# GregVS/Racing-SLAM

Measured on AMD Instinct MI355X. Metric: match+triangulate+local-BA passes/sec @ 2k kpts/frame, 20-KF×10k-pt window, higher is better.
Workload: dtype u8 Hamming (match), f64 (DLT SVD, BA), f32 (gates)

## Files before the change

racing-slam_amd/csrc/ba_solve_body.h:

```cpp
#pragma once
#include "ba_common.h"
#include "ba_backsub_body.h"

#define K7_THREADS 512
#ifndef K7_CHAIN_SIMDS
#define K7_CHAIN_SIMDS 1
#endif
#ifndef K7_V2
#define K7_V2 0
#endif
#if K7_CHAIN_SIMDS == 2
#define K7_TPW 9
#define K7_NTW 4
#else
#define K7_TPW 6
#define K7_NTW 6
#endif

typedef __attribute__((ext_vector_type(4))) double d4;

__device__ __forceinline__ double readlane_f64(double v, int lane)
{
    const int lo = __builtin_amdgcn_readlane(__double2loint(v), lane);
    const int hi = __builtin_amdgcn_readlane(__double2hiint(v), lane);
    return __hiloint2double(hi, lo);
}

__device__ __forceinline__ double fast_rcp(double x)
{
    double r = __builtin_amdgcn_rcp(x);
    const double e = fma(-x, r, 1.0);
    return fma(r, e, r);
}


template <bool HANDOFF, bool ROUND = false>
static __device__ __forceinline__ void ba_reduced_solve_lds_body(const BaDims& d, const BaBufs& b, const BaOpt& opt, const int it = 0,
                                                                 const int n_items = 0)
{
    extern __shared__ __attribute__((aligned(16))) double sm[];
    const int n = d.n, tid = threadIdx.x, nt = K7_THREADS;
    const int set = blockIdx.x;
    const int LD = n + 1 + ((n & 1) ? 1 : 0);
    double* A = sm;
    double* lam = A + (size_t)(n + 1) * LD;
    double* xs = lam + n;
    double* Minv = xs + n;
    double* Us = Minv + 6 * n;
    double* gcs = Us + 6 * n;
    double* grs = gcs + n;
    double* Pd = sm + (((size_t)(n + 1) * LD + 17 * (size_t)n + 1) & ~(size_t)1);
    double* Nf = Pd + 8 * 128;
    __shared__ BaState st;
    __shared__ int s_fail;
    __shared__ double red[K7_THREADS / 64];
    __shared__ double red3[K7_THREADS / 64][3];
    BA_STAMP_DECL;
    const int lane = tid & 63;
    const int wave = __builtin_amdgcn_readfirstlane(tid >> 6);
    const int lr = lane & 15, lq = lane >> 4;
    const int NTL = (n + 1 + 15) / 16;
#if K7_CHAIN_SIMDS == 2
    const bool chain = wave < 2;
    const bool idle = wave == 4 || wave == 5;
    const int tw = (wave & 1) + 2 * (wave >> 2);
    const int cw = wave;
#elif K7_V2
    const bool chain = (wave & 3) == 0;
    const bool idle = false;
    const int tw = chain ? 0 : wave - 1 - (wave >> 2);
#else
    const bool chain = (wave & 3) == 0;
    const bool idle = false;
    const int tw = chain ? 0 : wave - 1 - (wave >> 2);
    const int cw = wave >> 2;
#endif
    int tr[K7_TPW], tc[K7_TPW];
    bool tv[K7_TPW];
#pragma unroll
    for (int s = 0; s < K7_TPW; s++) {
        const int t = K7_NTW * s + tw;
        int r = 0;
#pragma unroll
        for (int q = 1; q < 8; q++) r += (t >= q * (q + 1) / 2) ? 1 : 0;
        tr[s] = r;
        tc[s] = t - r * (r + 1) / 2;
        tv[s] = !chain && !idle && r < NTL;
    }

    auto acc_ld = [&](const double* p) -> double { return ROUND ? ba_load_sc1(p) : *p; };
    if (ROUND) {
#if RS_STAMPS
        if (tid == 0 && set == 0) b.dbg[45] = wall_clock64();
#endif
        if (tid == 0) s_fail = 0;
        const BaState s0 = ba_round_state(b, opt, it, &st, set == 0);
        if (s0.done || set >= s0.nact) return;
        __shared__ unsigned s_lost;
        if (tid == 0) {
            const unsigned long long want = (unsigned long long)(unsigned)s0.n_rounds * (unsigned long long)n_items;
            const unsigned long long t0 = wall_clock64();
            unsigned lost = 0;
            while (ba_load_word_sc1(b.dbg + BA_SDONE) < want) {
                if (wall_clock64() - t0 > b.hand_timeout) { lost = 1; break; }
                __builtin_amdgcn_s_sleep(2);
            }
            s_lost = lost;
#if RS_STAMPS
            if (set == 0) b.dbg[44] = wall_clock64();
#endif
        }
        __syncthreads();
        if (s_lost) {
            if (tid == 0) {
                atomicAdd(b.dbg + BA_HAND_ERR, 1ull);
                const unsigned long long w = ((unsigned long long)(unsigned)s0.n_rounds << 2) | 2ull;
                ba_store_word_sc1(b.dbg + BA_HAND_TAKEN + set, w);
            }
            return;
        }
    }
    if (!ROUND && tid == 0) { st = *b.st; s_fail = 0; }
    double pre_cost = 0.0, pre_fail = 0.0, pre_gm = 0.0;
    if (tid < 64) {
        pre_cost = acc_ld(&b.scal[(size_t)tid * BA_SLOT_STRIDE + 0]);
        pre_fail = acc_ld(&b.scal[(size_t)tid * BA_SLOT_STRIDE + 1 + set]);
        for (int r = 0; r < b.gmax_blocks; r++)
            pre_gm = fmax(pre_gm, acc_ld(&b.gmax_all[((size_t)r * BA_NSLOT + tid) * BA_SLOT_STRIDE]));
    }
    const double pre_sc = tid < n ? b.sc[tid] : 1.0;
    double fold[2] = {0.0, 0.0}, keep[2] = {0.0, 0.0};
#pragma unroll
    for (int h = 0; h < 2; h++) {
        const int i = tid + h * nt;
        if (i < 8 * n) {
            const size_t addr = i < n ? (size_t)set * n + i : (size_t)(b.ns - 1) * n + i;
#pragma unroll
            for (int r = 0; r < BA_UREP; r++) fold[h] += acc_ld(&b.rhs[(size_t)r * b.cam_stride + addr]);
            if (i >= n) keep[h] = b.Ukeep[i - n];
        }
    }
    double sv[K7_TPW][4];
#pragma unroll
    for (int s = 0; s < K7_TPW; s++) {
#pragma unroll
        for (int q = 0; q < 4; q++) sv[s][q] = 0.0;
        if (!tv[s]) continue;
        const int kc = min(16 * tc[s] + lr, n - 1);
#pragma unroll
        for (int q = 0; q < 4; q++) {
            const int ic = min(16 * tr[s] + lq + 4 * q, n - 1);
            const double* sp = b.S + ((size_t)set * n + kc) * n + ic;
            double v = acc_ld(sp);
            for (int r = 1; r < b.srep; r++) v += acc_ld(sp + (size_t)r * b.s_rep_stride);
            sv[s][q] = v;
        }
    }
    __syncthreads();
    if (st.done || set >= st.nact) return;
#if RS_STAMPS
    if (HANDOFF && tid == 0 && set == 0) b.dbg[42] = wall_clock64();
#endif
    const unsigned long long epoch = (unsigned long long)(unsigned)st.n_rounds << 2;
    auto publish = [&](int word, unsigned long long code) {
        if (HANDOFF) {
            asm volatile("s_waitcnt vmcnt(0)" ::: "memory");
            __syncthreads();
            if (tid == 0) {
#if RS_STAMPS
                if (set == 0) b.dbg[word == BA_HAND ? 40 : 43] = wall_clock64();
#endif
                ba_store_word_sc1(b.dbg + word + set, epoch | code);
            }
        }
    };
    BA_STAMP(b, 2);
    for (int i = tid; i < BA_NSLOT * BA_SLOT_STRIDE; i += nt) {
        double* z = b.pt_scal + (size_t)set * BA_NSLOT * BA_SLOT_STRIDE + i;
        if (HANDOFF) ba_store_sc1(z, 0.0);
        else *z = 0.0;
    }
    for (int i = tid; i < 2 * 8 * 128; i += nt) Pd[i] = 0.0;
#if K7_V2
    for (int i = tid; i < (n + 1) * LD; i += nt) A[i] = 0.0;
#endif
#pragma unroll
    for (int h = 0; h < 2; h++) {
        const int i = tid + h * nt;
        if (i < 8 * n) {
            const double v = (i < n || st.fresh) ? fold[h] : keep[h];
            if (i >= n && st.fresh && set == 0) b.Ukeep[i - n] = v;
            if (i < n) grs[i] = v;
            else if (i < n + 6 * n) Us[i - n] = v;
            else gcs[i - 7 * n] = v;
        }
    }
    __syncthreads();
    for (int i = tid; i < n; i += nt) grs[i] += gcs[i];
    if (tid < n) {
        const double h = Us[(tid / 6) * 36 + (tid % 6) * 7];
        double sc = pre_sc;
        if (!st.have_scale) {
            sc = opt.jacobi ? 1.0 / (1.0 + sqrt(h)) : 1.0;
            if (set == 0) b.sc[tid] = sc;
        }
        const double s2 = sc * sc;
        lam[tid] = clampd(s2 * h, opt.dmin, opt.dmax) / (ba_set_radius(st, set) * s2);
    }
    BA_STAMP(b, 3);

    const double fail_sum = wave_sum(pre_fail);
    if (st.fresh) {
        const double c = wave_sum(pre_cost);
        const double gslots = wave_max_nonneg(pre_gm);
        double gm = 0.0;
        for (int i = tid; i < n; i += nt) gm = fmax(gm, fabs(gcs[i]));
        gm = wave_max_nonneg(gm);
        if ((tid & 63) == 0) red[tid >> 6] = gm;
        __syncthreads();
        if (tid == 0) {
            st.x_cost = c;
            if (st.iter == 0) st.initial_cost = st.x_cost;
            double g = gslots;
            for (int w = 0; w < nt / 64; w++) g = fmax(g, red[w]);
            if (!isfinite(st.x_cost)) { st.done = 1; st.termination = RS_BA_FAILURE; }
            else if (g <= opt.gtol) { st.done = 1; st.termination = RS_BA_CONVERGENCE_GRADIENT; }
        }
        __syncthreads();
        if (st.done) { if (tid == 0 && set == 0) *b.st = st; publish(BA_HAND_TAKEN, 2ull); return; }
    } else {
        __syncthreads();
    }
    publish(BA_HAND_TAKEN, 0ull);
    if (tid == 0 && fail_sum > 0.0) s_fail = 1;
    BA_STAMP(b, 0);

    const int NB = n / 6;
#if K7_V2
#if K7_V2 == 2
#define K7_RING(J_) ((J_) % 3)
#else
#define K7_RING(J_) 0
#endif
    double* const Dg0 = Pd;
    double* const Pds0 = Pd + 108;
    double* const ddv = Pd + 216;
    volatile int* const dflag = (volatile int*)(Pd + 232);
    volatile int* const cflag = dflag + 2;
    volatile int* const tflag = dflag + 4;
    auto wait_for = [&](volatile int* word, int want) {
        int spins = 0;
        while (*word < want) {
            if (++spins > (1 << 20)) { s_fail = 1; break; }
            __builtin_amdgcn_s_sleep(1);
        }
    };
    if (chain) {
        BA_STAMP(b, 1);
        const int sl = wave >> 2;
        const int i = 64 * sl + lane, ic = min(i, n);
        double Fp[6];
#pragma unroll
        for (int e = 0; e < 6; e++) Fp[e] = 0.0;
#if RS_STAMPS
        const unsigned long long cpre_ = wall_clock64();
#endif
        __syncthreads();
#if RS_STAMPS
        if (tid == 0 && blockIdx.x == 0) b.dbg[22] += wall_clock64() - cpre_;
#endif
#if RS_STAMPS >= 2
        unsigned long long cs_[6] = {0, 0, 0, 0, 0, 0}, ct_ = wall_clock64();
#define K7_CSTAMP(i) do { if (tid == 0 && blockIdx.x == 0) { const unsigned long long t__ = wall_clock64(); cs_[i] += t__ - ct_; ct_ = t__; } } while (0)
#else
#define K7_CSTAMP(i) do { } while (0)
#endif
        for (int J = 0; J < NB; J++) {
            const int c0 = 6 * J, r0 = c0 + 6;
            double* const Dg = Dg0 + 36 * K7_RING(J);
            double* const Pds = Pds0 + 36 * K7_RING(J);
            const double* const Pdp = Pds0 + 36 * K7_RING(J + 2);
            if (64 * sl + 63 < c0 || 64 * sl > n) {
#if K7_V2 == 2
                if (lane == 0) cflag[sl] = NB + 1;
                break;
#else
                __syncthreads();
                continue;
#endif
            }
#if K7_V2 == 2
            {
                const int other = sl ^ 1;
#pragma unroll
                for (int t = 0; t < K7_NTW; t++) wait_for(tflag + t, J);
                const bool other_owns = (c0 >> 6) == other || ((c0 + 5) >> 6) == other;
                wait_for(cflag + other, other_owns ? J : J - 1);
                __builtin_amdgcn_fence(__ATOMIC_ACQUIRE, "wavefront");
            }
#endif
            double x[6];
#pragma unroll
            for (int k = 0; k < 6; k++) x[k] = A[ic * LD + c0 + k];
            if (J > 0) {
                const double2* g2 = reinterpret_cast<const double2*>(Pdp);
#pragma unroll
                for (int e = 0; e < 6; e++) {
                    const double2 g01 = g2[3 * e], g23 = g2[3 * e + 1], g45 = g2[3 * e + 2];
                    x[0] -= Fp[e] * g01.x; x[1] -= Fp[e] * g01.y; x[2] -= Fp[e] * g23.x;
                    x[3] -= Fp[e] * g23.y; x[4] -= Fp[e] * g45.x; x[5] -= Fp[e] * g45.y;
                }
            }
            K7_CSTAMP(0);
            {
                const int a = i - c0;
                const int o_lo = c0 >> 6, o_hi = (c0 + 5) >> 6;
                if (a >= 0 && a < 6) {
#pragma unroll
                    for (int k = 0; k < 6; k++) Dg[a * 6 + k] = x[k];
                }
                if (sl == o_lo || sl == o_hi) {
                    __builtin_amdgcn_fence(__ATOMIC_RELEASE, "wavefront");
                    __builtin_amdgcn_s_waitcnt(0xc07f);
                    if (lane == 0) dflag[sl] = J + 1;
                }
                const int other = sl ^ 1;
                if (other == o_lo || other == o_hi) {
                    while (dflag[other] < J + 1) { }
                }
                __builtin_amdgcn_fence(__ATOMIC_ACQUIRE, "wavefront");
                __builtin_amdgcn_s_waitcnt(0xc07f);
            }
            double Lm[6][6];
#pragma unroll
            for (int a = 0; a < 6; a++)
#pragma unroll
                for (int e = 0; e <= a; e++) Lm[a][e] = Dg[a * 6 + e];
            K7_CSTAMP(1);
            double dinv[6], dpiv[6];
            bool fbad = false;
#pragma unroll
            for (int c = 0; c < 6; c++) {
                const double piv = Lm[c][c];
                if (!(piv > 0.0) || !isfinite(piv)) fbad = true;
                const double rd = fast_rcp(piv);
                dinv[c] = rd;
                dpiv[c] = piv;
                double lc[6];
#pragma unroll
                for (int a = c + 1; a < 6; a++) lc[a] = Lm[a][c] * rd;
#pragma unroll
                for (int a = c + 1; a < 6; a++)
#pragma unroll
                    for (int e = c + 1; e <= a; e++) Lm[a][e] -= lc[a] * Lm[e][c];
#pragma unroll
                for (int a = c + 1; a < 6; a++) Lm[a][c] = lc[a];
            }
            K7_CSTAMP(2);
            double F[6];
            {
                double t[6];
#pragma unroll
                for (int r = 0; r < 6; r++) {
                    double sacc = x[r];
#pragma unroll
                    for (int e = 0; e < r; e++) sacc -= t[e] * Lm[r][e];
                    t[r] = sacc;
                }
#pragma unroll
                for (int r = 0; r < 6; r++) F[r] = t[r] * dinv[r];
            }
            K7_CSTAMP(3);
            if (i >= c0 && i <= n) {
#pragma unroll
                for (int r = 0; r < 6; r++) A[i * LD + c0 + r] = F[r];
            }
            if (J + 1 < NB) {
                const int k0 = i - r0;
                if (k0 >= 0 && k0 < 6) {
#pragma unroll
                    for (int e = 0; e < 6; e++) Pds[e * 6 + k0] = F[e] * dpiv[e];
                }
                if (lane == 0 && sl == (c0 >> 6)) {
#pragma unroll
                    for (int e = 0; e < 6; e++) ddv[(J & 1) * 8 + e] = dpiv[e];
                }
            }
#pragma unroll
            for (int e = 0; e < 6; e++) Fp[e] = F[e];
            if (lane == 0 && fbad) s_fail = 1;
            K7_CSTAMP(4);
#if K7_V2 == 2
            __builtin_amdgcn_fence(__ATOMIC_RELEASE, "wavefront");
            __builtin_amdgcn_s_waitcnt(0xc07f);
            if (lane == 0) cflag[sl] = J + 1;
#else
            __syncthreads();
#endif
            K7_CSTAMP(5);
        }
#if K7_V2 == 2
        if (lane == 0 && cflag[sl] < NB) cflag[sl] = NB + 1;
#endif
#if RS_STAMPS >= 2
        if (tid == 0 && blockIdx.x == 0) { for (int q = 0; q < 6; q++) b.dbg[16 + q] += cs_[q]; }
#endif
#if RS_STAMPS
        if (tid == 0 && blockIdx.x == 0) { const unsigned long long t__ = wall_clock64(); b.dbg[30] += t__ - cpre_; b.dbg[23] = t__; b.dbg[31] += 1ull; }
#endif
    } else {
        d4 acc[K7_TPW];
#pragma unroll
        for (int s = 0; s < K7_TPW; s++) {
            acc[s] = d4{0.0, 0.0, 0.0, 0.0};
            if (!tv[s]) continue;
            const int k = 16 * tc[s] + lr;
            if (tr[s] >= tc[s] + 2 && 16 * tr[s] + 15 < n) {
#pragma unroll
                for (int q = 0; q < 4; q++) acc[s][q] = (k < n) ? sv[s][q] : 0.0;
                continue;
            }
            const int kc = min(k, n - 1), kb = kc / 6;
            const double gv = grs[kc];
#pragma unroll
            for (int q = 0; q < 4; q++) {
                const int i = 16 * tr[s] + lq + 4 * q;
                const int ic = min(i, n - 1);
                const double uv = Us[kb * 36 + (kc - 6 * kb) * 6 + ic % 6];
                double val = sv[s][q] + ((kb == ic / 6) ? uv : 0.0) + ((i == k) ? lam[ic] : 0.0);
                val = (k < n && i < n && k <= i) ? val : ((i == n && k < n) ? gv : 0.0);
                acc[s][q] = val;
            }
        }
        int paddr[K7_TPW];
        unsigned pmask[K7_TPW];
#pragma unroll
        for (int s = 0; s < K7_TPW; s++) {
            const int k = 16 * tc[s] + lr;
            paddr[s] = (16 * tr[s] + lq) * LD + k;
            unsigned m = 0;
#pragma unroll
            for (int q = 0; q < 4; q++) {
                const int i = 16 * tr[s] + lq + 4 * q;
                m |= (i >= k && i <= n) ? (1u << q) : 0u;
            }
            pmask[s] = m;
        }
        const int LD4 = 4 * LD;
#pragma unroll
        for (int s = 0; s < K7_TPW; s++) {
            if (!tv[s] || tc[s] != 0) continue;
            if (lr >= 6) continue;
#pragma unroll
            for (int q = 0; q < 4; q++)
                if (pmask[s] >> q & 1) A[paddr[s] + q * LD4] = acc[s][q];
        }
        int arow[K7_TPW], brow[K7_TPW];
#pragma unroll
        for (int s = 0; s < K7_TPW; s++) { arow[s] = min(16 * tr[s] + lr, n) * LD; brow[s] = min(16 * tc[s] + lr, n) * LD; }
        const int e1 = min(4 + lq, 5);
        const bool pad1 = lq >= 2;
        __syncthreads();
        for (int J = 0; J < NB; J++) {
            const int c0 = 6 * J, r0 = c0 + 6;
            if (J > 0) {
#if K7_V2 == 2
                wait_for(cflag + 0, J);
                wait_for(cflag + 1, J);
                __builtin_amdgcn_fence(__ATOMIC_ACQUIRE, "wavefront");
#endif
                const int cm = c0 - 6;
                const double* dv = ddv + ((J - 1) & 1) * 8;
                const double d0 = dv[lq], d1 = dv[4 + lq];
#pragma unroll
                for (int s = 0; s < K7_TPW; s++) {
                    if (!tv[s] || 16 * tc[s] + 15 < c0) continue;
                    const double a0 = A[arow[s] + cm + lq], a1 = A[arow[s] + cm + e1];
                    const double b0 = A[brow[s] + cm + lq], b1 = A[brow[s] + cm + e1];
                    acc[s] = __builtin_amdgcn_mfma_f64_16x16x4f64(-a0, b0 * d0, acc[s], 0, 0, 0);
                    acc[s] = __builtin_amdgcn_mfma_f64_16x16x4f64(pad1 ? 0.0 : -a1, b1 * d1, acc[s], 0, 0, 0);
                }
            }
            if (J + 1 < NB) {
#pragma unroll
                for (int s = 0; s < K7_TPW; s++) {
                    if (!tv[s] || 16 * tc[s] + 15 < r0 || 16 * tc[s] >= r0 + 6) continue;
                    const int k = 16 * tc[s] + lr;
                    if (k < r0 || k >= r0 + 6) continue;
#pragma unroll
                    for (int q = 0; q < 4; q++)
                        if (pmask[s] >> q & 1) A[paddr[s] + q * LD4] = acc[s][q];
                }
            }
#if K7_V2 == 2
            __builtin_amdgcn_fence(__ATOMIC_RELEASE, "wavefront");
            __builtin_amdgcn_s_waitcnt(0xc07f);
            if (lane == 0) tflag[tw] = J + 1;
#else
            __syncthreads();
#endif
        }
    }
#else
    if (chain) {
        BA_STAMP(b, 1);
        const int crow = cw * 64 + lane;
#if RS_STAMPS
        const unsigned long long cpre_ = wall_clock64();
#endif
        __syncthreads();
#if RS_STAMPS
        if (tid == 0 && blockIdx.x == 0) b.dbg[22] += wall_clock64() - cpre_;
#endif
        for (int J = 0; J < NB; J++) {
            const int c0 = 6 * J, r0 = c0 + 6;
            const int irow = r0 + crow;
            const bool has_row = irow <= n;
            if (wave != 0 && r0 + 64 > n) {
                __syncthreads();
                __syncthreads();
                continue;
            }
            double* row = A + min(irow, n) * LD + c0;
            double L[6][6], rr[6];
#pragma unroll
            for (int a = 0; a < 6; a++)
#pragma unroll
                for (int e = 0; e <= a; e++) L[a][e] = A[(c0 + a) * LD + c0 + e];
#pragma unroll
            for (int e = 0; e < 6; e++) rr[e] = row[e];
            double dinv[6], dpiv[6], F[6];
            bool fbad = false;
#pragma unroll
            for (int c = 0; c < 6; c++) {
                const double piv = L[c][c];
                if (!(piv > 0.0) || !isfinite(piv)) fbad = true;
                const double rd = fast_rcp(piv);
                dinv[c] = rd;
                dpiv[c] = piv;
                double lc[6];
#pragma unroll
                for (int a = c + 1; a < 6; a++) lc[a] = L[a][c] * rd;
#pragma unroll
                for (int a = c + 1; a < 6; a++)
#pragma unroll
                    for (int e = c + 1; e <= a; e++) L[a][e] -= lc[a] * L[e][c];
#pragma unroll
                for (int a = c + 1; a < 6; a++) L[a][c] = lc[a];
            }
            {
                double t[6];
#pragma unroll
                for (int r = 0; r < 6; r++) {
                    double sacc = rr[r];
#pragma unroll
                    for (int e = 0; e < r; e++) sacc -= t[e] * L[r][e];
                    t[r] = sacc;
                }
#pragma unroll
                for (int r = 0; r < 6; r++) F[r] = t[r] * dinv[r];
            }
            if (has_row) {
#pragma unroll
                for (int r = 0; r < 6; r++) {
                    row[r] = F[r];
                    Nf[r * 128 + irow] = -F[r];
                    Pd[r * 128 + irow] = F[r] * dpiv[r];
                }
            }
            __syncthreads();
            if (J + 1 < NB) {
                double* nxt = row + 6;
                double x[6];
#pragma unroll
                for (int k = 0; k < 6; k++) x[k] = nxt[k];
#pragma unroll
                for (int e = 0; e < 6; e++) {
                    const double2* g2 = reinterpret_cast<const double2*>(Pd + e * 128 + r0);
                    const double2 g01 = g2[0], g23 = g2[1], g45 = g2[2];
                    x[0] -= F[e] * g01.x; x[1] -= F[e] * g01.y;
                    x[2] -= F[e] * g23.x; x[3] -= F[e] * g23.y;
                    x[4] -= F[e] * g45.x; x[5] -= F[e] * g45.y;
                }
                if (has_row) {
#pragma unroll
                    for (int k = 0; k < 6; k++) nxt[k] = x[k];
                }
            }
            if (tid == 63) {
#pragma unroll
                for (int a = 1; a < 6; a++)
#pragma unroll
                    for (int e = 0; e < a; e++) Minv[J * 36 + a * 6 + e] = L[a][e];
                if (fbad) s_fail = 1;
            }
            __syncthreads();
        }
#if RS_STAMPS
        if (tid == 0 && blockIdx.x == 0) { const unsigned long long t__ = wall_clock64(); b.dbg[30] += t__ - cpre_; b.dbg[23] = t__; b.dbg[31] += 1ull; }
#endif
    } else {
        d4 acc[K7_TPW];
        double opA[K7_TPW][2], opB[K7_TPW][2];
#pragma unroll
        for (int s = 0; s < K7_TPW; s++) {
            acc[s] = d4{0.0, 0.0, 0.0, 0.0};
            opA[s][0] = opA[s][1] = opB[s][0] = opB[s][1] = 0.0;
            if (!tv[s]) continue;
            const int k = 16 * tc[s] + lr;
            if (tr[s] >= tc[s] + 2 && 16 * tr[s] + 15 < n) {
#pragma unroll
                for (int q = 0; q < 4; q++) acc[s][q] = (k < n) ? sv[s][q] : 0.0;
                continue;
            }
            const int kc = min(k, n - 1), kb = kc / 6;
            const double gv = grs[kc];
#pragma unroll
            for (int q = 0; q < 4; q++) {
                const int i = 16 * tr[s] + lq + 4 * q;
                const int ic = min(i, n - 1);
                const double uv = Us[kb * 36 + (kc - 6 * kb) * 6 + ic % 6];
                double val = sv[s][q] + ((kb == ic / 6) ? uv : 0.0) + ((i == k) ? lam[ic] : 0.0);
                val = (k < n && i < n && k <= i) ? val : ((i == n && k < n) ? gv : 0.0);
                acc[s][q] = val;
            }
        }
#pragma unroll
        for (int s = 0; s < K7_TPW; s++) {
            if (!tv[s] || tc[s] != 0) continue;
            const int k = lr;
            if (k >= 6) continue;
#pragma unroll
            for (int q = 0; q < 4; q++) {
                const int i = 16 * tr[s] + lq + 4 * q;
                if (i >= k && i <= n) A[i * LD + k] = acc[s][q];
            }
        }
        int paddr[K7_TPW];
        unsigned pmask[K7_TPW];
#pragma unroll
        for (int s = 0; s < K7_TPW; s++) {
            const int k = 16 * tc[s] + lr;
            paddr[s] = (16 * tr[s] + lq) * LD + k;
            unsigned m = 0;
#pragma unroll
            for (int q = 0; q < 4; q++) {
                const int i = 16 * tr[s] + lq + 4 * q;
                m |= (i >= k && i <= n) ? (1u << q) : 0u;
            }
            pmask[s] = m;
        }
        const int LD4 = 4 * LD;
        __syncthreads();
        for (int J = 0; J < NB; J++) {
            const int c0 = 6 * J, r0 = c0 + 6;
            if (J > 0) {
#pragma unroll
                for (int s = 1; s < K7_TPW; s += 2) {
                    if (!tv[s] || 16 * tc[s] + 15 < c0) continue;
                    acc[s] = __builtin_amdgcn_mfma_f64_16x16x4f64(opA[s][0], opB[s][0], acc[s], 0, 0, 0);
                    acc[s] = __builtin_amdgcn_mfma_f64_16x16x4f64(opA[s][1], opB[s][1], acc[s], 0, 0, 0);
                }
            }
            if (J + 1 < NB) {
#pragma unroll
                for (int s = 0; s < K7_TPW; s++) {
                    if (!tv[s] || 16 * tc[s] + 15 < r0 || 16 * tc[s] >= r0 + 6) continue;
                    const int k = 16 * tc[s] + lr;
                    if (k < r0 || k >= r0 + 6) continue;
#pragma unroll
                    for (int q = 0; q < 4; q++)
                        if (pmask[s] >> q & 1) A[paddr[s] + q * LD4] = acc[s][q];
                }
            }
            __syncthreads();
            if (J + 1 < NB) {
#pragma unroll
                for (int s = 0; s < K7_TPW; s++) {
                    if (!tv[s] || 16 * tc[s] + 15 < r0) continue;
#pragma unroll
                    for (int kc = 0; kc < 2; kc++) {
                        opA[s][kc] = Nf[(4 * kc + lq) * 128 + 16 * tr[s] + lr];
                        opB[s][kc] = Pd[(4 * kc + lq) * 128 + 16 * tc[s] + lr];
                    }
                }
#pragma unroll
                for (int s = 0; s < K7_TPW; s += 2) {
                    if (!tv[s] || 16 * tc[s] + 15 < r0) continue;
                    acc[s] = __builtin_amdgcn_mfma_f64_16x16x4f64(opA[s][0], opB[s][0], acc[s], 0, 0, 0);
                    acc[s] = __builtin_amdgcn_mfma_f64_16x16x4f64(opA[s][1], opB[s][1], acc[s], 0, 0, 0);
                }
            }
            __syncthreads();
        }
    }
#endif
    __syncthreads();
    if (s_fail) {
        if (tid == 0) {
            if (set == 0) { st.solver_failed = 1; *b.st = st; }
            else b.set_out[set].solver_failed = 1;
        }
        publish(BA_HAND, 1ull);
        return;
    }
    if (wave == 0) {
        const double* yrow = A + (size_t)n * LD;
        double y0 = yrow[min(lane, n)], y1 = yrow[min(64 + lane, n)];
        const int i0 = min(lane, n), i1 = min(64 + lane, n);
#define K7_BS_LOAD(J_, L_, P0_, P1_)                                                                       \
    {                                                                                                      \
        const int jj_ = max((J_), 0), cc_ = 6 * jj_;                                                       \
        _Pragma("unroll") for (int e = 1; e < 6; e++)                                                      \
            _Pragma("unroll") for (int t = 0; t < e; t++) L_[e][t] = K7_V2 ? A[(cc_ + e) * LD + cc_ + t] : Minv[jj_ * 36 + e * 6 + t]; \
        _Pragma("unroll") for (int e = 0; e < 6; e++) P0_[e] = A[(cc_ + e) * LD + i0];                     \
        if (cc_ > 64) { _Pragma("unroll") for (int e = 0; e < 6; e++) P1_[e] = A[(cc_ + e) * LD + i1]; }   \
    }
#define K7_BS_STEP(J_, L_, P0_, P1_)                                                                       \
    {                                                                                                      \
        const int c0_ = 6 * (J_);                                                                          \
        double x[6];                                                                                       \
        _Pragma("unroll") for (int t = 5; t >= 0; t--) {                                                   \
            const int idx = c0_ + t;                                                                       \
            double sacc = readlane_f64(idx >= 64 ? y1 : y0, idx & 63);                                     \
            _Pragma("unroll") for (int e = 5; e > t; e--) sacc -= L_[e][t] * x[e];                         \
            x[t] = sacc;                                                                                   \
        }                                                                                                  \
        _Pragma("unroll") for (int e = 0; e < 6; e++) y0 -= P0_[e] * x[e];                                 \
        if (c0_ > 64) { _Pragma("unroll") for (int e = 0; e < 6; e++) y1 -= P1_[e] * x[e]; }               \
        if (lane == 0) { _Pragma("unroll") for (int t = 0; t < 6; t++) xs[c0_ + t] = x[t]; }               \
    }
        double La[6][6], Pa0[6], Pa1[6], Lb[6][6], Pb0[6], Pb1[6];
        K7_BS_LOAD(NB - 1, La, Pa0, Pa1);
        for (int J = NB - 1; J >= 0; J -= 2) {
            K7_BS_LOAD(J - 1, Lb, Pb0, Pb1);
            K7_BS_STEP(J, La, Pa0, Pa1);
            if (J - 1 >= 0) {
                K7_BS_LOAD(J - 2, La, Pa0, Pa1);
                K7_BS_STEP(J - 1, Lb, Pb0, Pb1);
            }
        }
#undef K7_BS_LOAD
#undef K7_BS_STEP
    }
    __syncthreads();
    BA_STAMP(b, 6);
#if RS_STAMPS
    if (tid == 0 && blockIdx.x == 0) { b.dbg[25] += wall_clock64() - b.dbg[23]; }
#endif
    double* dc_set = b.dc + (size_t)set * BA_DC_STRIDE(n);
    if (HANDOFF) {
        int badi = 0;
        for (int i = tid; i < n; i += nt) {
            const double dlt = -xs[i];
            if (!isfinite(dlt)) badi = 1;
            ba_store_sc1(&dc_set[i], dlt);
        }
        publish(BA_HAND, __syncthreads_or(badi) ? 1ull : 0ull);
    }
    double mcc = 0.0, ssq = 0.0, xsq = 0.0;
    bool bad = false;
    const double* Xc = b.Xc + (size_t)st.cur * d.C * 6;
    const int cand = (st.cur + 1 + set) % (b.ns + 1);
    double* Xn = b.Xc + (size_t)cand * d.C * 6;
    for (int c = tid; c < d.C; c += nt) {
        const int s = b.slot[c];
        bool active = false;
        if (s >= 0)
            for (int k = 0; k < 6; k++) active = active || Us[s * 36 + k * 7] > 0.0;
        for (int k = 0; k < 6; k++) {
            const double x = Xc[6 * c + k];
            if (s >= 0) {
                const double dlt = -xs[6 * s + k];
                if (!isfinite(dlt)) bad = true;
                mcc += 0.5 * (dlt * dlt * lam[6 * s + k] - dlt * gcs[6 * s + k]);
                const double xn = x + dlt;
                if (active) { ssq += (x - xn) * (x - xn); xsq += x * x; }
                Xn[6 * c + k] = xn;
                if (!HANDOFF) dc_set[6 * s + k] = dlt;
            } else {
                Xn[6 * c + k] = x;
            }
        }
        cam_prepare(Xn + 6 * c, b.prep + ((size_t)cand * d.C + c) * BA_PREP);
    }
    mcc = wave_sum(mcc); ssq = wave_sum(ssq); xsq = wave_sum(xsq);
    if (__any(bad) && (tid & 63) == 0) s_fail = 1;
    if ((tid & 63) == 0) { red3[tid >> 6][0] = mcc; red3[tid >> 6][1] = ssq; red3[tid >> 6][2] = xsq; }
    __syncthreads();
    if (tid == 0) {
        double a0 = 0, a1 = 0, a2 = 0;
        for (int w = 0; w < nt / 64; w++) { a0 += red3[w][0]; a1 += red3[w][1]; a2 += red3[w][2]; }
        if (set == 0) {
            st.cam_scal[0] = a0; st.cam_scal[1] = a1; st.cam_scal[2] = a2;
            st.solver_failed = s_fail;
            *b.st = st;
        } else {
            BaSetOut so;
            so.cam_scal[0] = a0; so.cam_scal[1] = a1; so.cam_scal[2] = a2; so.cam_scal[3] = 0.0;
            so.solver_failed = s_fail;
#pragma unroll
            for (int q = 0; q < 7; q++) so.pad[q] = 0;
            b.set_out[set] = so;
        }
    }
    BA_STAMP(b, 7);
    BA_STAMP_FLUSH(b, 0);
}
```

Before: 1998.

## Precompute block-scaled off-diagonal columns in parallel before single-wave back-substitution

```diff
diff --git a/racing-slam_amd/csrc/ba_solve_body.h b/racing-slam_amd/csrc/ba_solve_body.h
--- a/racing-slam_amd/csrc/ba_solve_body.h
+++ b/racing-slam_amd/csrc/ba_solve_body.h
@@ -704,44 +704,78 @@
         publish(BA_HAND, 1ull);
         return;
     }
+    for (int idx = tid; idx < NB * (n + 1); idx += nt) {
+        const int J = idx / (n + 1), c = idx - J * (n + 1), c0 = 6 * J;
+        if (c < c0 + 6) continue;
+        double q[6];
+#pragma unroll
+        for (int a = 0; a < 6; a++) q[a] = A[c * LD + c0 + a];
+#pragma unroll
+        for (int a = 4; a >= 0; a--)
+#pragma unroll
+            for (int e = 5; e > a; e--) q[a] -= (K7_V2 ? A[(c0 + e) * LD + c0 + a] : Minv[J * 36 + e * 6 + a]) * q[e];
+#pragma unroll
+        for (int a = 0; a < 6; a++) A[(c0 + a) * LD + c] = q[a];
+    }
+    __syncthreads();
     if (wave == 0) {
-        const double* yrow = A + (size_t)n * LD;
-        double y0 = yrow[min(lane, n)], y1 = yrow[min(64 + lane, n)];
-        const int i0 = min(lane, n), i1 = min(64 + lane, n);
-#define K7_BS_LOAD(J_, L_, P0_, P1_)                                                                       \
+        const double* q0row = A + (size_t)min(lane, n) * LD;
+        const double* q1row = A + (size_t)min(64 + lane, n) * LD;
+        double x0 = q0row[n], x1 = q1row[n];
+#define K7_BS_LOAD(K_, Q0_, Q1_)                                                                           \
     {                                                                                                      \
-        const int jj_ = max((J_), 0), cc_ = 6 * jj_;                                                       \
-        _Pragma("unroll") for (int e = 1; e < 6; e++)                                                      \
-            _Pragma("unroll") for (int t = 0; t < e; t++) L_[e][t] = K7_V2 ? A[(cc_ + e) * LD + cc_ + t] : Minv[jj_ * 36 + e * 6 + t]; \
-        _Pragma("unroll") for (int e = 0; e < 6; e++) P0_[e] = A[(cc_ + e) * LD + i0];                     \
-        if (cc_ > 64) { _Pragma("unroll") for (int e = 0; e < 6; e++) P1_[e] = A[(cc_ + e) * LD + i1]; }   \
-    }
-#define K7_BS_STEP(J_, L_, P0_, P1_)                                                                       \
+        const int c_ = 6 * max((K_), 0);                                                                   \
+        _Pragma("unroll") for (int e = 0; e < 6; e++) Q0_[e] = q0row[c_ + e];                              \
+        if (c_ > 64) { _Pragma("unroll") for (int e = 0; e < 6; e++) Q1_[e] = q1row[c_ + e]; }             \
+    }
+#define K7_BS_STEP(K_, Q0_, Q1_, HI_)                                                                      \
     {                                                                                                      \
-        const int c0_ = 6 * (J_);                                                                          \
-        double x[6];                                                                                       \
-        _Pragma("unroll") for (int t = 5; t >= 0; t--) {                                                   \
-            const int idx = c0_ + t;                                                                       \
-            double sacc = readlane_f64(idx >= 64 ? y1 : y0, idx & 63);                                     \
-            _Pragma("unroll") for (int e = 5; e > t; e--) sacc -= L_[e][t] * x[e];                         \
-            x[t] = sacc;                                                                                   \
+        const int c0_ = 6 * (K_);                                                                          \
+        double xk[6];                                                                                      \
+        _Pragma("unroll") for (int e = 0; e < 6; e++)                                                      \
+            xk[e] = readlane_f64((HI_) == 1 || ((HI_) == 2 && e >= 4) ? x1 : x0, (c0_ + e) & 63);          \
+        const double t0_ = (Q0_[0] * xk[0] + Q0_[1] * xk[1] + Q0_[2] * xk[2]) + (Q0_[3] * xk[3] + Q0_[4] * xk[4] + Q0_[5] * xk[5]); \
+        if ((HI_) == 1) {                                                                                  \
+            const double t1_ = (Q1_[0] * xk[0] + Q1_[1] * xk[1] + Q1_[2] * xk[2]) + (Q1_[3] * xk[3] + Q1_[4] * xk[4] + Q1_[5] * xk[5]); \
+            x0 -= t0_;                                                                                     \
+            x1 = 64 + lane < c0_ ? x1 - t1_ : x1;                                                          \
+        } else {                                                                                           \
+            x0 = lane < c0_ ? x0 - t0_ : x0;                                                               \
         }                                                                                                  \
-        _Pragma("unroll") for (int e = 0; e < 6; e++) y0 -= P0_[e] * x[e];                                 \
-        if (c0_ > 64) { _Pragma("unroll") for (int e = 0; e < 6; e++) y1 -= P1_[e] * x[e]; }               \
-        if (lane == 0) { _Pragma("unroll") for (int t = 0; t < 6; t++) xs[c0_ + t] = x[t]; }               \
-    }
-        double La[6][6], Pa0[6], Pa1[6], Lb[6][6], Pb0[6], Pb1[6];
-        K7_BS_LOAD(NB - 1, La, Pa0, Pa1);
-        for (int J = NB - 1; J >= 0; J -= 2) {
-            K7_BS_LOAD(J - 1, Lb, Pb0, Pb1);
-            K7_BS_STEP(J, La, Pa0, Pa1);
-            if (J - 1 >= 0) {
-                K7_BS_LOAD(J - 2, La, Pa0, Pa1);
-                K7_BS_STEP(J - 1, Lb, Pb0, Pb1);
+    }
+        double Qa0[6], Qa1[6], Qb0[6], Qb1[6];
+        int K = NB - 1;
+        if (K >= 11) {
+            K7_BS_LOAD(K, Qa0, Qa1);
+            for (;;) {
+                K7_BS_LOAD(K - 1, Qb0, Qb1);
+                K7_BS_STEP(K, Qa0, Qa1, 1);
+                if (--K < 11) break;
+                K7_BS_LOAD(K - 1, Qa0, Qa1);
+                K7_BS_STEP(K, Qb0, Qb1, 1);
+                if (--K < 11) break;
+            }
+        }
+        if (K == 10) {
+            K7_BS_LOAD(10, Qa0, Qa1);
+            K7_BS_STEP(10, Qa0, Qa1, 2);
+            K = 9;
+        }
+        if (K >= 1) {
+            K7_BS_LOAD(K, Qa0, Qa1);
+            for (;;) {
+                K7_BS_LOAD(K - 1, Qb0, Qb1);
+                K7_BS_STEP(K, Qa0, Qa1, 0);
+                if (--K < 1) break;
+                K7_BS_LOAD(K - 1, Qa0, Qa1);
+                K7_BS_STEP(K, Qb0, Qb1, 0);
+                if (--K < 1) break;
             }
         }
 #undef K7_BS_LOAD
 #undef K7_BS_STEP
+        if (lane < n) xs[lane] = x0;
+        if (64 + lane < n) xs[64 + lane] = x1;
     }
     __syncthreads();
     BA_STAMP(b, 6);
```

Result: no change. 2015, median of 6 (+0.8%).
